# pierlj/ken-burns-effect

Measured on AMD Instinct MI355X. Metric: novel_view_frames_per_sec_1024x1024, higher is better.
Workload: dtype f32; 1 GPU; 1024x1024 KBE path, 1137109 pts (inpaint cloud), frame=shift+scatter+fill+u8+crop/resize; delivery=pinned_host, scatter_route=fused, frames_per_rank=1589, lanes=2, device_only_lanes=4, warmup_frames=3178, passes=1, handoff=sdma, ranks_seen=1

## Files before the change

### include/kbe.h

```cpp
#ifndef KBE_H
#define KBE_H

#include <stddef.h>
#include <stdint.h>

#ifdef __cplusplus
extern "C" {
#endif

#define KBE_ABI_VERSION 11

#if defined(__GNUC__)
#define KBE_API __attribute__((visibility("default")))
#else
#define KBE_API
#endif

enum {
    KBE_OK = 0,
    KBE_E_INVALID = -1,
    KBE_E_LAUNCH = -2,
    KBE_E_DEVICE = -3
};

// ... 87 lines not shown
                                         const double* focals, const float* shifts, void* const* scratch, uint8_t* const* frames_u8,
                                         const int* turns, int placed, int n_next, const double* next_focals, const float* next_shifts,
                                         void* const* next_scratch, const int* next_turns, int stages, const int* fill_rect,
                                         double near_depth, kbe_stream_t stream);

KBE_API int kbe_render_pointcloud_tiled(const float* points, const float* data, int N, int C, int W, int H, double focal,
                                        double baseline, const float* shift3, void* scratch, float* render,
                                        float* existing, kbe_stream_t stream);

#define KBE_MAX_LANES 8
KBE_API size_t kbe_video_scratch_stride(int W, int H, int N);
KBE_API size_t kbe_video_stage_bytes(int W, int H, int lanes, int batch);
#define KBE_VIDEO_FILL_DIST 1
#define KBE_VIDEO_FILL_GROUP(n) (((n) - 1) << 1)
#define KBE_VIDEO_GROUP(n) (((n) - 1) << 5)
#define KBE_VIDEO_FREE_TRANSFERS 8
#define KBE_VIDEO_EVEN_GROUPS 16
#define KBE_VIDEO_NO_AHEAD 512
#define KBE_VIDEO_FAST_RAMP 1024
#define KBE_VIDEO_SDMA 8192
#define KBE_VIDEO_FUSED_LEAN 2048
#define KBE_VIDEO_FUSED_ROOMY 4096
#define KBE_VIDEO_FILL_PAIRS KBE_VIDEO_FILL_GROUP(2)
#define KBE_VIDEO_INJECT_FAULT 32768
#define KBE_VIDEO_INJECT_TIMEOUT 65536
KBE_API int kbe_render_video(const float* points, const float* image, const float* depth, int N, int W, int H,
                             double baseline, int n_frames, const double* focals, const float* shifts, int crop_w,
                             int crop_h, void* scratch, uint8_t* stage, int batch, uint8_t* host_out,
                             int raster_w, int raster_n, const void* packed, double cloud_focal, int flags,
                             kbe_stream_t stream, kbe_stream_t copy_stream, int lanes, const kbe_stream_t* lane_streams,
                             double near_depth);
KBE_API int kbe_video_handoff_status(void);

KBE_API int kbe_generate_mask(const float* points, const float* shift, int B, int N, int W, int H, double focal,
                              double baseline, unsigned long long* keys, int32_t* winner, float* masks, float* zee,
                              int32_t* ids, kbe_stream_t stream);

KBE_API int kbe_frame_u8(const float* render_chw, int W, int H, uint8_t* frame_hwc, kbe_stream_t stream);

KBE_API int kbe_crop_resize_u8(const uint8_t* frame_hwc, int W, int H, int crop_w, int crop_h,
                       uint8_t* out_hwc, kbe_stream_t stream);


KBE_API int kbe_depth_to_points(const float* depth, const float* valid, int B, int W, int H, double focal,
                        float* points, kbe_stream_t stream);

// ... 27 lines not shown
```

### ken-burns-effect_amd/_native.py

```python
import ctypes
import os

import torch

_HERE = os.path.dirname(os.path.abspath(__file__))
LIB_PATH = os.environ.get('KBE_LIB_PATH') or os.path.join(_HERE, 'csrc', 'libkbe_hip.so')

SYMBOLS = (
    'kbe_abi_version', 'kbe_last_error', 'kbe_device_info', 'kbe_selftest_err', 'kbe_selftest_division', 'kbe_zkeys_clear', 'kbe_zsplat', 'kbe_zkeys_decode',
    'kbe_degrid', 'kbe_degrid_serial', 'kbe_accumulate', 'kbe_normalize', 'kbe_render_pointcloud', 'kbe_fill_disocclusion',
    'kbe_frame_scratch_bytes', 'kbe_frame_scratch_init', 'kbe_render_frame', 'kbe_render_frame_stages', 'kbe_render_frame_group', 'kbe_cloud_pack_bytes', 'kbe_cloud_pack', 'kbe_render_frame_fused', 'kbe_render_frame_group_fused', 'kbe_render_frame_group_ahead_ok', 'kbe_render_frame_group_ahead', 'kbe_video_scratch_stride', 'kbe_video_stage_bytes', 'kbe_render_video', 'kbe_render_pointcloud_tiled', 'kbe_generate_mask', 'kbe_frame_u8', 'kbe_crop_resize_u8', 'kbe_depth_to_points', 'kbe_shift_points',
    'kbe_spatial_filter', 'kbe_laplacian_valid', 'kbe_pconv_epilogue', 'kbe_prelu_mask', 'kbe_bias_act', 'kbe_upsample2x_act', 'kbe_frame_scratch_init_sets', 'kbe_video_handoff_status',
)

ABI_VERSION = 11
MAX_LANES = 8
DEFAULT_LANES = 4
FUSED_MAX_DENSITY = 20.0
FUSED_MAX_POINTS = 1 << 28
FUSED_DENSE = 1.5
FUSED_HOST_GROUP = 12
DEFAULT_FILL_GROUP = 4
PROBE_MIN_FRAMES = 128
DEFAULT_HOST_LANES = 2
# ... 516 lines not shown
        if 'stage' not in state or state['stage'].numel() < need:
            state['stage'] = torch.empty(need, dtype=torch.uint8, device=dev)
        if 'copy_stream' not in state:
            state['copy_stream'] = torch.cuda.Stream(device=dev)
            state['lane_streams'] = [None] + lane_streams_of(dev, state['lanes'] - 1)
        lane_streams = (ctypes.c_void_p * MAX_LANES)(*[None if st is None else st.cuda_stream for st in state['lane_streams']])
        focals = (ctypes.c_double * max(n, 1))(*[float(c[0]) for c in cameras])
        shifts = (ctypes.c_float * max(3 * n, 1))(*[float(v) for c in cameras for v in c[1]])
        cw, ch = (0, 0) if crop is None else (int(crop[0]), int(crop[1]))
        copy_stream = ctypes.c_void_p(state['copy_stream'].cuda_stream) if overlap else _stream()
        flags, group, fused = self.video_launch_shape(state, cameras, batch, to_host=not host_out.is_cuda)
        base_flags = flags
        if fused:
            self._pack(state)
        free = os.environ.get('KBE_FREE_TRANSFERS', 'auto')
        if not host_out.is_cuda and (free == '1' or (free == 'auto' and flags & 1)):
            flags |= 8
        if os.environ.get('KBE_EVEN_GROUPS') == '1':
            flags |= 16
        if os.environ.get('KBE_RAMP', 'classic') == 'fast':
            flags |= 1024
        if os.environ.get('KBE_AHEAD') == '0':
            flags |= 512
        flags |= fused_build_bits(video=True)
        if not host_out.is_cuda and batch < 0 and handoff_by_sdma():
            flags |= 8192
            if os.environ.get('KBE_INJECT_HANDOFF_FAULT') == '1':
                flags |= 32768
            if os.environ.get('KBE_INJECT_HANDOFF_TIMEOUT') == '1':
                flags |= 65536
        keep_flags = flags & ~base_flags
        scratch = state['scratch']
        if group > 1:
            fits = group
            if 'scratch_groups' not in state or state['scratch_groups'].numel() < group * lanes * self.scratch_stride(state) or os.environ.get('KBE_SCRATCH_BUDGET_MB'):
                max_sets = self.scratch_set_budget(state)
                while fits > 1 and fits * lanes > max_sets:
                    fits = max(1, fits // 2)
            if fits != group:
                flags, group, fused = self.video_launch_shape(state, cameras, batch, to_host=not host_out.is_cuda, max_group=fits)
                flags |= keep_flags
        state['video_sets'] = group * lanes
        if group > 1:
            scratch, _ = self.group_scratch(state, group * lanes)
        self._check(self.lib.kbe_render_video(_ptr(state['points']), _ptr(state['image']), _ptr(state['depth']), _i(state['N']),
                                              _i(W), _i(H), _d(float(baseline)), _i(n), focals, shifts, _i(cw), _i(ch),
# ... 183 lines not shown
```

### ken-burns-effect_amd/csrc/kbe_fill.h

```cpp
#pragma once
#include <hip/hip_runtime.h>
#include <math.h>

#pragma clang fp contract(off)

namespace kbe {

struct FillDirs { float x[16], y[16]; };

inline FillDirs make_fill_dirs()
{
    const float dx[16] = { -1, 0, 1, 1, -1, 1, 2, 2, -2, -1, 1, 2, 3, 3, 3, 3 };
    const float dy[16] = { 1, 1, 1, 0, 2, 2, 1, -1, 3, 3, 3, 3, 2, 1, -1, -2 };
    FillDirs d;
    for (int i = 0; i < 16; i++) {
        volatile float n = sqrtf((dx[i] * dx[i]) + (dy[i] * dy[i]));
        d.x[i] = dx[i] / n;
        d.y[i] = dy[i] / n;
    }
    return d;
}

template <class DepthAt>
__device__ __forceinline__ int fill_source(const FillDirs& dirs, int x, int y, int W, int H, DepthAt depth_at)
{
// ... 14 lines not shown
        if ((iax < 0) | (iax >= W) | (iay < 0) | (iay >= H)) continue;
        float bx = (float) x, by = (float) y;
        int ibx, iby;
        float db = 0.0f;
        for (;;) {
            bx += ddx; ibx = (int) roundf(bx);
            by += ddy; iby = (int) roundf(by);
            if ((ibx < 0) | (ibx >= W) | (iby < 0) | (iby >= H)) break;
            db = depth_at(ibx, iby);
            if (db > 0.0f) break;
        }
        if ((ibx < 0) | (ibx >= W) | (iby < 0) | (iby >= H)) continue;
        const float ex = (float) (ibx - iax), ey = (float) (iby - iay);
        const float dist = sqrtf(ex * ex + ey * ey);
        if (shortest > dist) {
            fx = iax; fy = iay;
            if (da < db) { fx = ibx; fy = iby; }
            shortest = dist;
        }
    }
    return (fx < 0 || fy < 0) ? -1 : fy * W + fx;
}


}
```

### ken-burns-effect_amd/csrc/kbe_frame.hip

```cpp
#include <stdlib.h>
#include <string.h>

#include <chrono>
#include <mutex>
#include <thread>
#include <vector>
#include <hsa/hsa.h>
#include <hsa/hsa_ext_amd.h>

#include "kbe_cloud.h"
#include "kbe_tiles.h"
#include "kbe_video_plan.h"

using namespace kbe;

namespace {

__global__ void k_scratch_init(uint32_t* zkeys, uint32_t* zkeys_b, size_t hw, int* tile_count, int n_tiles, int* hole_count)
{
    const size_t stride = (size_t) gridDim.x * blockDim.x, gtid = (size_t) blockIdx.x * blockDim.x + threadIdx.x;
    for (size_t i = gtid; i < hw; i += stride) { zkeys[i] = KBE_ZKEY_EMPTY; if (zkeys_b) zkeys_b[i] = KBE_ZKEY_EMPTY; }
    for (size_t i = gtid; i < (size_t) n_tiles; i += stride) { tile_count[i * CNT_STRIDE] = 0; tile_count[i * CNT_STRIDE + 1] = 0; }
    if (gtid < (size_t) HOLE_COUNT_INTS) hole_count[gtid] = 0;
}
// ... 1194 lines not shown
        const hipError_t e = hipMemsetAsync(stage + ctl_offset, 0, sizeof(DeliverCtl), cs);
        if (e != hipSuccess) return fail(KBE_E_LAUNCH, "kbe_render_video: hipMemsetAsync", e);
    }
    if (packed) {
        const Scratch sc0 = carve(scratch, W, H);
        hipLaunchKernelGGL(k_zero_counters, dim3(16, group * lanes), dim3(256), 0, cs, sc0.hole_count, sb, group * lanes, sc0.tile_count,
                           2 * align16(4 * (size_t) sc0.tiles_x * sc0.tiles_y * CNT_STRIDE) / sizeof(int));
        if (int rc0 = launched("kbe_render_video/counters")) return rc0;
    }
    hipEvent_t start = lanes > 1 || (ringed && dc != cs) ? make() : nullptr;
    if (start && ok) {
        (void) hipEventRecord(start, cs);
        for (int l = 1; l < lanes; l++) (void) hipStreamWaitEvent(ls[l], start, 0);
        if (ringed && dc != cs) (void) hipStreamWaitEvent(dc, start, 0);
    }
    const VideoPlan plan = plan_video(VideoPlanIn{ n_frames, lanes, group, batch, dest, fin, (flags & KBE_VIDEO_FAST_RAMP) != 0, (flags & KBE_VIDEO_EVEN_GROUPS) != 0,
                                                   packed != nullptr, !(flags & KBE_VIDEO_NO_AHEAD) },
                                      [&](int n, int n_next) { return fused_can_place_ahead(N, W, H, n, n_next); });

    static const FillDirs fill_dirs = make_fill_dirs();
    const int in_flight = plan.single ? lanes : lanes * group;
    const int fill_flags = in_flight >= KBE_FILL_BY_COUNT_MIN_LANES ? (KBE_STAGE_FILL_BY_COUNT | ((flags & KBE_VIDEO_FILL_DIST) ? KBE_STAGE_FILL_DIST : 0)) : 0;
    const int build = (flags & KBE_VIDEO_FUSED_LEAN) ? 1 : ((flags & KBE_VIDEO_FUSED_ROOMY) ? 2 : 0);
    auto dst = [&](const PlanFrame& f) { return (dest == VideoDest::HBM ? host_out : ringed ? ring0 : finished) + (size_t) f.slot * fb; };
    auto fused_target = [&](const PlanFrame& f, uint8_t* frame) {
        char* const scr = (char*) scratch + (size_t) f.set * sb;
        return FusedTarget{ make_camera(W, H, focals[f.frame], baseline, shifts + 3 * (size_t) f.frame), carve(scr, W, H), scratch_place(scr, W, H), f.turn & 1, frame,
                            nullptr, nullptr, nullptr, nullptr, f.turn };
    };
    auto render = [&](const PlanLaunch& a) {
        const hipStream_t s = ls[a.lane];
        const PlanFrame* const fr = &plan.frames[a.first];
        uint8_t* outs[KBE_FRAME_JOBS];
        uint8_t* raws[KBE_FRAME_JOBS];
        for (int j = 0; j < a.count; j++) {
            outs[j] = dst(fr[j]);
            raws[j] = crop ? stage + (size_t) (KBE_FRAME_JOBS * a.lane + j) * fb : outs[j];
        }
        int rc = KBE_OK;
        if (!packed) {
            FrameJob jobs[KBE_FILL_JOBS];
            for (int j = 0; j < a.count; j++)
                jobs[j] = FrameJob{ focals[fr[j].frame], shifts + 3 * (size_t) fr[j].frame, (char*) scratch + (size_t) fr[j].set * sb, raws[j], nullptr, nullptr, nullptr, nullptr,
                                    fr[j].zbuf == PLAN_ZBUF_A ? KBE_STAGE_ZBUF_A : (fr[j].zbuf == PLAN_ZBUF_B ? KBE_STAGE_ZBUF_B : 0) };
            rc = render_jobs(points, image, depth, N, W, H, baseline, a.count, jobs, KBE_VIDEO_STAGES | fill_flags, crop ? rect : nullptr, raster_w, raster_n, s);
        } else if (plan.single) {
            rc = kbe_render_frame_fused(packed, N, cloud_focal, W, H, focals[fr[0].frame], baseline, shifts + 3 * (size_t) fr[0].frame, (char*) scratch + (size_t) fr[0].set * sb,
                                        raws[0], nullptr, nullptr, nullptr, nullptr, KBE_STAGE_TILES | KBE_STAGE_FILL | fill_flags |
                                        ((flags & KBE_VIDEO_FUSED_LEAN) ? KBE_STAGE_FUSED_LEAN : 0) | ((flags & KBE_VIDEO_FUSED_ROOMY) ? KBE_STAGE_FUSED_ROOMY : 0),
                                        crop ? rect : nullptr, fr[0].turn & 1, (kbe_stream_t) s);
        } else {
            FusedTarget ft[KBE_FRAME_JOBS], nt[KBE_FRAME_JOBS];
            FillTarget targets[KBE_FRAME_JOBS];
            for (int j = 0; j < a.count; j++) {
                ft[j] = fused_target(fr[j], raws[j]);
                targets[j] = FillTarget{ ft[j].sc, ft[j].sc.hole_count + (fr[j].turn & 1), raws[j], nullptr, 0, ft[j].sc.hole_count + ((fr[j].turn & 1) ^ 1) };
            }
            const int n_next = a.next >= 0 ? plan.launches[a.next].count : 0;
            for (int j = 0; j < n_next; j++) nt[j] = fused_target(plan.frames[plan.launches[a.next].first + j], nullptr);
            launch_frames_fused(s, a.count, packed, N, cloud_focal, ft, a.placed, n_next, nt, build, near_depth);
            if ((rc = launched("kbe_render_video/scatter"))) return rc;
            const FillRect fr_rect = { rect[0], rect[1], rect[2], rect[3] };
            for (int j0 = 0; j0 < a.count; j0 += KBE_FILL_JOBS)
                launch_fill(s, a.count - j0 < KBE_FILL_JOBS ? a.count - j0 : KBE_FILL_JOBS, targets + j0, W, H, KBE_STAGE_FILL | fill_flags, fill_dirs, fr_rect,
                            targets[0].sc.tiles_x * targets[0].sc.tiles_y);
            rc = launched("kbe_render_video/fill");
        }
        for (int j0 = 0; j0 < a.count && rc == KBE_OK && crop; j0 += KBE_FILL_JOBS)
            rc = crop_resize_group(a.count - j0 < KBE_FILL_JOBS ? a.count - j0 : KBE_FILL_JOBS, raws + j0, W, H, crop_w, crop_h, outs + j0, s);
        return rc;
    };

    DeliverCtl* const ctl_turns = host_dev && lanes > 1 && !(flags & KBE_VIDEO_FREE_TRANSFERS) ? (DeliverCtl*) (stage + ctl_offset) : nullptr;
    SdmaCall sdma;
    bool sdma_asked = !(flags & KBE_VIDEO_SDMA);
    volatile int64_t* lane_fin[KBE_MAX_LANES] = {};
    const double group_us = (double) -batch * (double) fb / 50.0e3;
    const int turn_polls = (int) fmin(fmax(3.0 * lanes * group_us, (double) DELIVER_MAX_POLLS), 1.0e6);
    hipEvent_t rendered[2][KBE_MAX_LANES] = {}, copied[2] = { nullptr, nullptr };
    for (int h = 0; h < 2 && ringed; h++) {
        copied[h] = make();
        for (int l = 0; l < lanes; l++) if (ls[l] != dc) rendered[h][l] = make();
    }
    if (dest == VideoDest::GROUPS) trace.start((int) plan.units.size(), cs);
    auto wait = [&](int u, const PlanUnit& un) {
        if (dest == VideoDest::GROUPS) {
            trace.begin(u, ls[un.lane]);
            if (lane_fin[un.lane]) hipLaunchKernelGGL(k_signal_wait, dim3(1), dim3(64), 0, ls[un.lane], lane_fin[un.lane], sdma_pool().wait_ticks, sdma_pool().gave_up);
// ... 102 lines not shown
```

### ken-burns-effect_amd/csrc/kbe_hip.hip

```cpp
#include <hip/hip_runtime.h>
#include <math.h>
#include <stdio.h>
#include <string.h>

#include "kbe.h"
#include "kbe_device.h"
#include "kbe_fill.h"
#include "kbe_host.h"

#pragma clang fp contract(off)

using namespace kbe;

thread_local char kbe::g_err[256] = "";

namespace {

__global__ void k_fill_u32(uint32_t* p, size_t n, uint32_t v)
{
    const size_t stride = (size_t) gridDim.x * blockDim.x;
    for (size_t i = (size_t) blockIdx.x * blockDim.x + threadIdx.x; i < n; i += stride) p[i] = v;
}

__global__ void k_zkeys_decode(const uint32_t* keys, size_t n, float* zee)
// ... 226 lines not shown
    s0 = min(max(s, 0), src_n - 1);
    s1 = min(max(s + 1, 0), src_n - 1);
    c0 = cv_round((1.f - f) * 2048.f);
    c1 = cv_round(f * 2048.f);
}

__device__ __forceinline__ uint32_t mul_u24_v(uint32_t a, uint32_t b) { uint32_t r; asm("v_mul_u32_u24 %0, %1, %2" : "=v"(r) : "v"(a), "v"(b)); return r; }
__device__ __forceinline__ uint32_t mad_u24_v(uint32_t a, uint32_t b, uint32_t c) { uint32_t r; asm("v_mad_u32_u24 %0, %1, %2, %3" : "=v"(r) : "v"(a), "v"(b), "v"(c)); return r; }
__device__ __forceinline__ uint32_t mul_u24_s(uint32_t a, uint32_t b) { uint32_t r; asm("v_mul_u32_u24 %0, %1, %2" : "=v"(r) : "s"(a), "v"(b)); return r; }
__device__ __forceinline__ uint32_t mul_hi_u24_s(uint32_t a, uint32_t b) { uint32_t r; asm("v_mul_hi_u32_u24 %0, %1, %2" : "=v"(r) : "s"(a), "v"(b)); return r; }
__device__ __forceinline__ uint32_t mad_u24_s(uint32_t a, uint32_t b, uint32_t c) { uint32_t r; asm("v_mad_u32_u24 %0, %1, %2, %3" : "=v"(r) : "s"(a), "v"(b), "v"(c)); return r; }

#ifndef KBE_CROP_TH
#define KBE_CROP_TH 16
#endif
constexpr int CR_TW = 64, CR_TH = KBE_CROP_TH, CR_THREADS = 256, CR_WAVES = CR_THREADS / 64;
constexpr int CR_ROWS_PER_WAVE = CR_TH / CR_WAVES;
constexpr int CR_PROWS = CR_TH + 2, CR_PCOLS = CR_TW + 2;
constexpr int CR_PBYTES = CR_PCOLS * 3, CR_PSTRIDE = (CR_PBYTES + 3) / 4 + 1;
constexpr int CR_RROWS = CR_PROWS + 1, CR_RDW = ((CR_PCOLS + 1) * 3 + 3 + 3) / 4 + 1;
constexpr int CR_STAGE = (CR_RROWS + CR_WAVES - 1) / CR_WAVES;
static_assert(CR_TH % CR_WAVES == 0 && CR_RDW <= 64 && CR_PBYTES <= CR_THREADS && CR_TW + CR_TH <= CR_THREADS && CR_PROWS + 1 <= CR_THREADS, "crop tile geometry");

__device__ __forceinline__ void crop_resize_body(const uint8_t* __restrict__ img, int W, int H, int cw, int ch_, double scale_x, double scale_y, uint8_t* __restrict__ out)
{
    __shared__ uint32_t s_raw[CR_RROWS][CR_RDW];
    __shared__ uint32_t s_patch[CR_PROWS][CR_PSTRIDE];
    __shared__ __attribute__((aligned(16))) uint32_t s_out[CR_TH][CR_TW * 3 / 4];
    __shared__ int s_cx[4][CR_TW], s_cy[4][CR_TH];
    __shared__ int s_ro[CR_PROWS + 1];
    const int tid = threadIdx.x;
    const int bx = blockIdx.x * CR_TW, by = blockIdx.y * CR_TH;
    const float cx = (float) W / 2.0f - (float) (cw - 1) * 0.5f, cy = (float) H / 2.0f - (float) (ch_ - 1) * 0.5f;
    const int ipx = (int) floorf(cx), ipy = (int) floorf(cy);
    const float fa = cx - (float) ipx, fb = cy - (float) ipy;
    const int a11 = cv_round((1.f - fa) * (1.f - fb) * 65536.f), a12 = cv_round(fa * (1.f - fb) * 65536.f);
    const int a21 = cv_round((1.f - fa) * fb * 65536.f), a22 = cv_round(fa * fb * 65536.f);
    const bool whole = (a12 | a21 | a22) == 0;
    if (tid < CR_TW + CR_TH) {
        const bool col = tid < CR_TW;
        const int k = col ? tid : tid - CR_TW;
        int s0, s1, c0, c1;
        if (col) resize_coeff(min(bx + k, W - 1), scale_x, cw, true, s0, s1, c0, c1);
        else resize_coeff(min(by + k, H - 1), scale_y, ch_, false, s0, s1, c0, c1);
        int* t = col ? &s_cx[0][k] : &s_cy[0][k];
        const int stride = col ? CR_TW : CR_TH;
        t[0] = s0; t[stride] = s1; t[2 * stride] = c0; t[3 * stride] = c1;
    }
    __syncthreads();
    const int px_lo = s_cx[0][0], px_hi = s_cx[1][CR_TW - 1], py_lo = s_cy[0][0], py_hi = s_cy[1][CR_TH - 1];
    const int n_pc3 = (px_hi - px_lo + 1) * 3, n_pr = py_hi - py_lo + 1;
    const int rx0 = min(max(ipx + px_lo, 0), W - 1), rx1 = min(max(ipx + px_hi + 1, 0), W - 1);
    const int ry0 = min(max(ipy + py_lo, 0), H - 1), ry1 = min(max(ipy + py_hi + 1, 0), H - 1);
    const int n_rows = ry1 - ry0 + 1;
    const size_t frame_bytes = (size_t) W * H * 3;
    const int wv = __builtin_amdgcn_readfirstlane(tid >> 6), ln = tid & 63;
    uint32_t stage[CR_STAGE];
#pragma unroll
    for (int k = 0; k < CR_STAGE; k++) {
        const int r = wv + CR_WAVES * k;
        stage[k] = 0;
        if (r < n_rows) {
            const size_t b0 = ((size_t) (ry0 + r) * W + rx0) * 3, b1 = ((size_t) (ry0 + r) * W + rx1) * 3 + 3;
            const size_t a0 = b0 & ~(size_t) 3;
            const int n_dw = (int) ((b1 - a0 + 3) >> 2);
            const uint8_t* row = img + a0;
            if (a0 + 4 * (size_t) n_dw <= frame_bytes) {
                if (ln < n_dw) stage[k] = ((const uint32_t*) row)[ln];
            } else if (ln < n_dw) {
                for (int t = 0; t < 4; t++) if (a0 + 4 * (size_t) ln + t < frame_bytes) stage[k] |= (uint32_t) row[4 * ln + t] << (8 * t);
            }
        }
    }
#pragma unroll
    for (int k = 0; k < CR_STAGE; k++) {
        const int r = wv + CR_WAVES * k;
        if (r < CR_RROWS && ln < CR_RDW) s_raw[r][ln] = stage[k];
    }
    if (tid <= CR_PROWS) {
        const int y = min(max(ipy + py_lo + tid, 0), H - 1);
        s_ro[tid] = min(y - ry0, CR_RROWS - 1) * (int) sizeof(s_raw[0]) + (int) ((((uint32_t) y * (uint32_t) W + (uint32_t) rx0) * 3u) & 3u);
    }
    __syncthreads();
    const uint8_t* raw = (const uint8_t*) s_raw;
    uint8_t* patch = (uint8_t*) s_patch;
    if (!whole) {
        if (tid < n_pc3) {
            const int pc = tid / 3, c = tid - pc * 3;
            const int x0 = (min(max(ipx + px_lo + pc, 0), W - 1) - rx0) * 3 + c, x1 = (min(max(ipx + px_lo + pc + 1, 0), W - 1) - rx0) * 3 + c;
            int o = s_ro[0];
            int t0 = raw[o + x0], t1 = raw[o + x1];
            for (int pr = 0; pr < n_pr; pr++) {
                o = s_ro[pr + 1];
                const int u0 = raw[o + x0], u1 = raw[o + x1];
                const uint32_t t = mad_u24_s((uint32_t) a22, (uint32_t) u1, mad_u24_s((uint32_t) a21, (uint32_t) u0, mad_u24_s((uint32_t) a12, (uint32_t) t1, mad_u24_s((uint32_t) a11, (uint32_t) t0, 1u << 15))));
                patch[pr * (int) sizeof(s_patch[0]) + tid] = (uint8_t) (t >> 16);
                t0 = u0; t1 = u1;
            }
        }
        __syncthreads();
    }
    const int col = tid & (CR_TW - 1);
    const uint8_t* const src = whole ? raw : (const uint8_t*) patch;
    int sx, sx1;
    if (whole) {
        sx = (min(max(ipx + s_cx[0][col], 0), W - 1) - rx0) * 3;
// ... 48 lines not shown
            if (by + r < H) ((uint4*) (out + ((size_t) (by + r) * W + bx) * 3))[k] = ((const uint4*) s_out[r])[k];
        }
    } else if ((W & 3) == 0 && bx + CR_TW <= W) {
        constexpr int DW = CR_TW * 3 / 4;
        for (int i = tid; i < CR_TH * DW; i += CR_THREADS) {
            const int r = i / DW, k = i - r * DW;
            if (by + r < H) ((uint32_t*) (out + ((size_t) (by + r) * W + bx) * 3))[k] = s_out[r][k];
        }
    } else {
#pragma unroll
        for (int m = 0; m < CR_ROWS_PER_WAVE; m++) {
            const int dx = bx + col, dy = by + wv * CR_ROWS_PER_WAVE + m;
            if (dx < W && dy < H) {
                const size_t o = ((size_t) dy * W + dx) * 3;
                out[o] = px[m][0]; out[o + 1] = px[m][1]; out[o + 2] = px[m][2];
            }
        }
    }
}

__global__ void __launch_bounds__(CR_THREADS) k_crop_resize_u8(const uint8_t* __restrict__ img, int W, int H, int cw, int ch_, double scale_x, double scale_y,
                                                               uint8_t* __restrict__ out)
{
    crop_resize_body(img, W, H, cw, ch_, scale_x, scale_y, out);
}

struct CropJobs { const uint8_t* img[4]; uint8_t* out[4]; };
__global__ void __launch_bounds__(CR_THREADS) k_crop_resize_u8_group(CropJobs jobs, int W, int H, int cw, int ch_, double scale_x, double scale_y)
{
    crop_resize_body(jobs.img[blockIdx.z], W, H, cw, ch_, scale_x, scale_y, jobs.out[blockIdx.z]);
}


__device__ __forceinline__ float linspace_centered(int n, int i)
{
    const float start = (float) ((-0.5 * n) + 0.5), end = (float) ((0.5 * n) - 0.5);
    if (n == 1) return start;
    const float step = (end - start) / (float) (n - 1);
    return (i < n / 2) ? start + step * (float) i : end - step * (float) (n - 1 - i);
}

__global__ void __launch_bounds__(kBlock) k_depth_to_points(const float* __restrict__ depth, const float* __restrict__ valid,
                                                            int W, int H, float inv_focal, float* __restrict__ points)
{
    const int b = blockIdx.y;
    const int HW = W * H;
    const int i = blockIdx.x * blockDim.x + threadIdx.x;
    if (i >= HW) return;
    const int y = i / W, x = i - y * W;
    float d = depth[(size_t) b * HW + i];
    if (valid) d = d * valid[(size_t) b * HW + i];
    const float u = linspace_centered(W, x) * inv_focal;
    const float v = linspace_centered(H, y) * inv_focal;
// ... 352 lines not shown
}

int kbe_crop_resize_u8(const uint8_t* frame_hwc, int W, int H, int crop_w, int crop_h, uint8_t* out_hwc,
                       kbe_stream_t stream)
{
    KBE_REQUIRE(frame_hwc && out_hwc && W > 0 && H > 0 && crop_w > 0 && crop_h > 0 && crop_w <= W && crop_h <= H,
                "kbe_crop_resize_u8: bad arguments");
    hipLaunchKernelGGL(k_crop_resize_u8, dim3((W + CR_TW - 1) / CR_TW, (H + CR_TH - 1) / CR_TH), dim3(CR_THREADS), 0,
                       (hipStream_t) stream, frame_hwc, W, H, crop_w, crop_h, (double) crop_w / W, (double) crop_h / H, out_hwc);
    return launched("kbe_crop_resize_u8");
}

}

namespace kbe {
int crop_resize_group(int n, const uint8_t* const* frames, int W, int H, int crop_w, int crop_h, uint8_t* const* outs, hipStream_t stream)
{
    if (n == 1) return kbe_crop_resize_u8(frames[0], W, H, crop_w, crop_h, outs[0], (kbe_stream_t) stream);
    CropJobs jobs;
    for (int k = 0; k < 4; k++) { jobs.img[k] = frames[k < n ? k : 0]; jobs.out[k] = outs[k < n ? k : 0]; }
    hipLaunchKernelGGL(k_crop_resize_u8_group, dim3((W + CR_TW - 1) / CR_TW, (H + CR_TH - 1) / CR_TH, n), dim3(CR_THREADS), 0, stream, jobs, W, H, crop_w, crop_h, (double) crop_w / W, (double) crop_h / H);
    return launched("kbe_crop_resize_u8 (group)");
}
}

extern "C" {

int kbe_depth_to_points(const float* depth, const float* valid, int B, int W, int H, double focal, float* points,
                        kbe_stream_t stream)
{
    KBE_REQUIRE(depth && points && B > 0 && W > 0 && H > 0, "kbe_depth_to_points: bad arguments");
    const float inv = (float) (1.0 / focal);
    hipLaunchKernelGGL(k_depth_to_points, dim3(blocks_for((size_t) W * H), B), dim3(kBlock), 0, (hipStream_t) stream, depth,
                       valid, W, H, inv, points);
    return launched("kbe_depth_to_points");
}

int kbe_shift_points(const float* points, int B, int N, const float* shift3, float* out, kbe_stream_t stream)
{
    KBE_REQUIRE(shift3 && B > 0 && N >= 0, "kbe_shift_points: bad arguments");
    if (N == 0) return KBE_OK;
    KBE_REQUIRE(points && out, "kbe_shift_points: points/out is NULL");
    const Camera cam = make_camera(1, 1, 1.0, 1.0, shift3);
    hipLaunchKernelGGL(k_shift_points, dim3(blocks_for(N), B), dim3(kBlock), 0, (hipStream_t) stream, points, N, cam, out);
    return launched("kbe_shift_points");
}
// ... 68 lines not shown
```

### ken-burns-effect_amd/csrc/kbe_holes.hip

```cpp
#include "kbe_tiles.h"

using namespace kbe;

namespace {


#ifndef KBE_FILL_SERIAL_BATCH
#define KBE_FILL_SERIAL_BATCH 8
#endif
constexpr int COARSE_WORDS = 2048;
#ifndef KBE_FILL_SERIAL_MIN
#define KBE_FILL_SERIAL_MIN 49152
#endif

__device__ __forceinline__ void fill_hole_serial(int px, const float* __restrict__ depth, const uint32_t* __restrict__ mask, int W, int H,
                                                 int wpr, const FillDirs& dirs, int bx0, int by0, int bx1, int by1,
                                                 uint8_t* __restrict__ frame, float* __restrict__ render,
                                                 const uint32_t* near, int c_wpr)
{
    constexpr int SB = KBE_FILL_SERIAL_BATCH;
    static_assert(SB <= 8, "a skipped batch must stay within one 8 x 8 block of where it ends");
    auto far_from_valid = [&](int px_, int py_) { return !((near[(py_ >> 3) * c_wpr + (px_ >> 8)] >> ((px_ >> 3) & 31)) & 1u); };
    const int y = px / W, x = px - y * W;
    float best = 1000000.0f;
// ... 412 lines not shown

#ifndef KBE_FILL_TABLES_BLOCKS
#define KBE_FILL_TABLES_BLOCKS 768
#endif
#ifndef KBE_FILL_BURST
#define KBE_FILL_BURST 4
#endif
#ifndef KBE_FILL_BURST_LANES
#define KBE_FILL_BURST_LANES 16
#endif
#ifndef KBE_FILL_REFILL_MIN
#define KBE_FILL_REFILL_MIN 16
#endif
#ifndef KBE_FILL_FINE_BELOW
#define KBE_FILL_FINE_BELOW 2
#endif
constexpr unsigned long long FILL_NO_ENTRY = ~0ull;
constexpr int FILL_MAX_STEPS = (1 << 14) - 1;
enum { END_IDLE = 0, END_WALK = 1, END_HIT = 2, END_DEAD = 3 };

__device__ __forceinline__ int swap_with_neighbour(int v)
{
    return __builtin_amdgcn_update_dpp(0, v, 0xB1, 0xF, 0xF, false);
}

__device__ __forceinline__ void valid_box(const int4* __restrict__ bbox, int n_tiles, int W, int H, int (*s_bb)[4], int& bx0, int& by0, int& bx1, int& by1)
{
    bx0 = W; by0 = H; bx1 = -1; by1 = -1;
    for (int t = threadIdx.x; t < n_tiles; t += blockDim.x) {
        const int4 bb = bbox[t];
        bx0 = min(bx0, bb.x); by0 = min(by0, bb.y); bx1 = max(bx1, bb.z); by1 = max(by1, bb.w);
    }
#pragma unroll
    for (int off = 32; off > 0; off >>= 1) {
        bx0 = min(bx0, __shfl_xor(bx0, off)); by0 = min(by0, __shfl_xor(by0, off));
        bx1 = max(bx1, __shfl_xor(bx1, off)); by1 = max(by1, __shfl_xor(by1, off));
    }
    if ((threadIdx.x & 63) == 0) { s_bb[threadIdx.x >> 6][0] = bx0; s_bb[threadIdx.x >> 6][1] = by0; s_bb[threadIdx.x >> 6][2] = bx1; s_bb[threadIdx.x >> 6][3] = by1; }
    __syncthreads();
    for (int w = 0; w < (int) (blockDim.x >> 6); w++) { bx0 = min(bx0, s_bb[w][0]); by0 = min(by0, s_bb[w][1]); bx1 = max(bx1, s_bb[w][2]); by1 = max(by1, s_bb[w][3]); }
}

#if defined(KBE_FILL_TABLES_WAVES)
#define KBE_FILL_TABLES_ATTR __attribute__((amdgpu_waves_per_eu(KBE_FILL_TABLES_WAVES, KBE_FILL_TABLES_WAVES)))
#else
#define KBE_FILL_TABLES_ATTR
#endif
__device__ __forceinline__ void fill_tables_body(const int* __restrict__ holes, const int* __restrict__ hole_count, int min_holes,
                                                     const float* __restrict__ depth, int W, int H, FillDirs dirs, FillRect rect,
                                                     uint8_t* __restrict__ frame, float* __restrict__ render, int n_tiles,
                                                     const int4* __restrict__ bbox, int tiles_x, int tiles_y,
                                                     const uint8_t* __restrict__ dist, const float2* __restrict__ strips,
                                                     const uint8_t* __restrict__ dist_blocks)
{
    const int n = min(*hole_count, W * H);
    if (n < min_holes || (int) (blockIdx.x * blockDim.x) >= n) return;
    __shared__ int s_bb[4][4];
    static_assert(KBE_DIST_CAP_BLOCKS <= 15, "block distances are stored in 4 bits");
    __shared__ uint32_t s_pool[COARSE_WORDS];
    int bx0, by0, bx1, by1;
    valid_box(bbox, n_tiles, W, H, s_bb, bx0, by0, bx1, by1);
    constexpr int FB = 256;
    static_assert(FB % 64 == 0 && FB * 16 <= 65536, "queue entries are 16 bits");
// ... 296 lines not shown
                }
                s_near[idx] = near;
            }
            __syncthreads();
        }
        const int gtid = blockIdx.x * blockDim.x + threadIdx.x, gsz = gridDim.x * blockDim.x;
        for (int h = gtid; h < n; h += gsz) {
            const int px = holes[h];
            const int y = px / W, x = px - y * W;
            if (x < rect.x0 || x > rect.x1 || y < rect.y0 || y > rect.y1) continue;
            fill_hole_serial(px, depth, mask, W, H, wpr, dirs, bx0, by0, bx1, by1, frame, render, skip_ok ? s_near : nullptr, c_wpr);
        }
        return;
    }
    const int lane = threadIdx.x & 31;
    const int group = (blockIdx.x * blockDim.x + threadIdx.x) >> 5, n_groups = (gridDim.x * blockDim.x) >> 5;
    const int d = lane >> 1, end = lane & 1;
    const float ddx = end ? dirs.x[d] : -dirs.x[d], ddy = end ? dirs.y[d] : -dirs.y[d];
    const size_t HW = (size_t) W * H;
    for (int h = group; h < n; h += n_groups) {
        const int px = holes[h];
        const int y = px / W, x = px - y * W;
        if (x < rect.x0 || x > rect.x1 || y < rect.y0 || y > rect.y1) continue;
        float fx = (float) x, fy = (float) y;
        int ix = 0, iy = 0;
        bool ok = false;
        bool done = (x < bx0 && ddx <= 0.0f) || (x > bx1 && ddx >= 0.0f) || (y < by0 && ddy <= 0.0f) || (y > by1 && ddy >= 0.0f);
        done = done || (bool) __shfl_xor((int) done, 1);
        auto walk = [&](auto batch_tag) {
            constexpr int kBatch = decltype(batch_tag)::value;
            int bx[kBatch], by[kBatch];
            uint32_t bw[kBatch];
            bool bin[kBatch];
#pragma unroll
            for (int k = 0; k < kBatch; k++) {
                fx += ddx; bx[k] = (int) roundf(fx);
                fy += ddy; by[k] = (int) roundf(fy);
                bin[k] = ((unsigned) bx[k] < (unsigned) W) & ((unsigned) by[k] < (unsigned) H);
                const unsigned mi = bin[k] ? (unsigned) by[k] * (unsigned) wpr + ((unsigned) bx[k] >> 5) : 0u;
                bw[k] = mask[mi];
            }
            bool stop = false;
#pragma unroll
            for (int k = 0; k < kBatch; k++) {
                const bool hit = bin[k] && ((bw[k] >> (bx[k] & 31)) & 1u);
                const bool take = !stop;
                ix = take ? bx[k] : ix; iy = take ? by[k] : iy;
                ok = ok || (take && hit);
                stop = stop || hit || !bin[k];
            }
            done = stop || (ix < bx0 && ddx <= 0.0f) || (ix > bx1 && ddx >= 0.0f) || (iy < by0 && ddy <= 0.0f) || (iy > by1 && ddy >= 0.0f);
        };
        int ox = 0, oy = 0;
        bool ook = false;
        float dist = INFINITY, best = INFINITY;
        for (;;) {
            if (!done) walk(std::integral_constant<int, 8>());
            ox = __shfl_xor(ix, 1); oy = __shfl_xor(iy, 1);
            ook = (bool) __shfl_xor((int) ok, 1);
            const bool odone = (bool) __shfl_xor((int) done, 1);
            const float ex = (float) (ix - ox), ey = (float) (iy - oy);
            const float cur = sqrtf(ex * ex + ey * ey);
            dist = (ok && ook && 1000000.0f > cur) ? cur : INFINITY;
            best = dist;
#pragma unroll
            for (int off = 2; off < 32; off <<= 1) best = fminf(best, __shfl_xor(best, off));
            done = done || (odone && !ook) || cur > best;
            if (__all(done)) break;
        }
        if (best == INFINITY) continue;
        const unsigned long long m = __ballot(dist == best);
        const unsigned mine = (unsigned) (m >> (threadIdx.x & 32));
        const int win = __ffs((int) mine) - 1;
        if (lane == win) {
            int sxp = ix, syp = iy;
            if (depth[(size_t) iy * W + ix] < depth[(size_t) oy * W + ox]) { sxp = ox; syp = oy; }
            const size_t s = (size_t) syp * W + sxp, o = (size_t) px;
            frame[o * 3] = frame[s * 3]; frame[o * 3 + 1] = frame[s * 3 + 1]; frame[o * 3 + 2] = frame[s * 3 + 2];
            if (render) for (int c = 0; c < 4; c++) render[c * HW + o] = render[c * HW + s];
        }
    }
}


}

namespace {

__global__ void __launch_bounds__(256) k_hole_dist(FillJobs jobs, int W, int H, int min_holes, int tiles_x, int tiles_y, FillDirs dirs, int image_rows, int use_strips)
{
    const FillJob& J = jobs.j[blockIdx.z];
    hole_dist_body(J.mask, W, H, J.dist, J.hole_count, min_holes, J.bbox, tiles_x, tiles_y, use_strips ? J.strips : nullptr, dirs, J.coarse, J.dist_blocks, image_rows);
}

__global__ void __launch_bounds__(256) KBE_FILL_TABLES_ATTR k_fill_tables(FillJobs jobs, int min_holes, int W, int H, FillDirs dirs, FillRect rect, int n_tiles,
                                                                         int tiles_x, int tiles_y, int use_strips)
{
    const FillJob& J = jobs.j[blockIdx.y];
    fill_tables_body(J.holes, J.hole_count, min_holes, J.depth, W, H, dirs, rect, J.frame, J.render, n_tiles, J.bbox, tiles_x, tiles_y, J.dist,
// ... 61 lines not shown
```

Measured before the change: 17800 frames/s.

## Fuse disocclusion fill into the crop-resize kernel for video frames

Adds a fused fill+crop/resize kernel. It gathers hole pixels from the validity mask into shared memory per tile, runs the half-wave ray walk to find a source pixel, and patches the staged raw rows before resampling. This replaces the separate fill kernel launch and its full-frame read-modify-write of the u8 frame when cropping is active. The walk logic is factored into a shared helper, and an env flag restores the old path. One risk is that fill sources are read from the unfilled image, so a hole filled from another hole may differ from the sequential path.

```diff
diff --git a/include/kbe.h b/include/kbe.h
--- a/include/kbe.h
+++ b/include/kbe.h
@@ -133,6 +133,7 @@
 #define KBE_VIDEO_FUSED_LEAN 2048
 #define KBE_VIDEO_FUSED_ROOMY 4096
 #define KBE_VIDEO_FILL_PAIRS KBE_VIDEO_FILL_GROUP(2)
+#define KBE_VIDEO_SEPARATE_FILL 16384
 #define KBE_VIDEO_INJECT_FAULT 32768
 #define KBE_VIDEO_INJECT_TIMEOUT 65536
 KBE_API int kbe_render_video(const float* points, const float* image, const float* depth, int N, int W, int H,
diff --git a/ken-burns-effect_amd/_native.py b/ken-burns-effect_amd/_native.py
--- a/ken-burns-effect_amd/_native.py
+++ b/ken-burns-effect_amd/_native.py
@@ -562,6 +562,8 @@
             flags |= 1024
         if os.environ.get('KBE_AHEAD') == '0':
             flags |= 512
+        if os.environ.get('KBE_FILL_CROP') == '0':
+            flags |= 16384
         flags |= fused_build_bits(video=True)
         if not host_out.is_cuda and batch < 0 and handoff_by_sdma():
             flags |= 8192
diff --git a/ken-burns-effect_amd/csrc/kbe_fill.h b/ken-burns-effect_amd/csrc/kbe_fill.h
--- a/ken-burns-effect_amd/csrc/kbe_fill.h
+++ b/ken-burns-effect_amd/csrc/kbe_fill.h
@@ -1,6 +1,8 @@
 #pragma once
 #include <hip/hip_runtime.h>
 #include <math.h>
+#include <stdint.h>
+#include <type_traits>
 
 #pragma clang fp contract(off)
 
@@ -61,5 +63,89 @@
     return (fx < 0 || fy < 0) ? -1 : fy * W + fx;
 }
 
+__device__ __forceinline__ void valid_box(const int4* __restrict__ bbox, int n_tiles, int W, int H, int (*s_bb)[4], int& bx0, int& by0, int& bx1, int& by1)
+{
+    bx0 = W; by0 = H; bx1 = -1; by1 = -1;
+    for (int t = threadIdx.x; t < n_tiles; t += blockDim.x) {
+        const int4 bb = bbox[t];
+        bx0 = min(bx0, bb.x); by0 = min(by0, bb.y); bx1 = max(bx1, bb.z); by1 = max(by1, bb.w);
+    }
+#pragma unroll
+    for (int off = 32; off > 0; off >>= 1) {
+        bx0 = min(bx0, __shfl_xor(bx0, off)); by0 = min(by0, __shfl_xor(by0, off));
+        bx1 = max(bx1, __shfl_xor(bx1, off)); by1 = max(by1, __shfl_xor(by1, off));
+    }
+    if ((threadIdx.x & 63) == 0) { s_bb[threadIdx.x >> 6][0] = bx0; s_bb[threadIdx.x >> 6][1] = by0; s_bb[threadIdx.x >> 6][2] = bx1; s_bb[threadIdx.x >> 6][3] = by1; }
+    __syncthreads();
+    for (int w = 0; w < (int) (blockDim.x >> 6); w++) { bx0 = min(bx0, s_bb[w][0]); by0 = min(by0, s_bb[w][1]); bx1 = max(bx1, s_bb[w][2]); by1 = max(by1, s_bb[w][3]); }
+}
+
+__device__ __forceinline__ bool halfwave_fill_source(int x, int y, float ddx, float ddy, const float* __restrict__ depth, const uint32_t* __restrict__ mask,
+                                                     int W, int H, int wpr, int bx0, int by0, int bx1, int by1, int& sx, int& sy)
+{
+    float fx = (float) x, fy = (float) y;
+    int ix = 0, iy = 0;
+    bool ok = false;
+    bool done = (x < bx0 && ddx <= 0.0f) || (x > bx1 && ddx >= 0.0f) || (y < by0 && ddy <= 0.0f) || (y > by1 && ddy >= 0.0f);
+    done = done || (bool) __shfl_xor((int) done, 1);
+    auto walk = [&](auto batch_tag) {
+        constexpr int kBatch = decltype(batch_tag)::value;
+        int bx[kBatch], by[kBatch];
+        uint32_t bw[kBatch];
+        bool bin[kBatch];
+#pragma unroll
+        for (int k = 0; k < kBatch; k++) {
+            fx += ddx; bx[k] = (int) roundf(fx);
+            fy += ddy; by[k] = (int) roundf(fy);
+            bin[k] = ((unsigned) bx[k] < (unsigned) W) & ((unsigned) by[k] < (unsigned) H);
+            const unsigned mi = bin[k] ? (unsigned) by[k] * (unsigned) wpr + ((unsigned) bx[k] >> 5) : 0u;
+            bw[k] = mask[mi];
+        }
+        bool stop = false;
+#pragma unroll
+        for (int k = 0; k < kBatch; k++) {
+            const bool hit = bin[k] && ((bw[k] >> (bx[k] & 31)) & 1u);
+            const bool take = !stop;
+            ix = take ? bx[k] : ix; iy = take ? by[k] : iy;
+            ok = ok || (take && hit);
+            stop = stop || hit || !bin[k];
+        }
+        done = stop || (ix < bx0 && ddx <= 0.0f) || (ix > bx1 && ddx >= 0.0f) || (iy < by0 && ddy <= 0.0f) || (iy > by1 && ddy >= 0.0f);
+    };
+    int ox = 0, oy = 0;
+    bool ook = false;
+    float dist = INFINITY, best = INFINITY;
+    for (;;) {
+        if (!done) walk(std::integral_constant<int, 8>());
+        ox = __shfl_xor(ix, 1); oy = __shfl_xor(iy, 1);
+        ook = (bool) __shfl_xor((int) ok, 1);
+        const bool odone = (bool) __shfl_xor((int) done, 1);
+        const float ex = (float) (ix - ox), ey = (float) (iy - oy);
+        const float cur = sqrtf(ex * ex + ey * ey);
+        dist = (ok && ook && 1000000.0f > cur) ? cur : INFINITY;
+        best = dist;
+#pragma unroll
+        for (int off = 2; off < 32; off <<= 1) best = fminf(best, __shfl_xor(best, off));
+        done = done || (odone && !ook) || cur > best;
+        if (__all(done)) break;
+    }
+    if (best == INFINITY) return false;
+    const unsigned long long m = __ballot(dist == best);
+    const unsigned mine = (unsigned) (m >> (threadIdx.x & 32));
+    const int win = __ffs((int) mine) - 1;
+    if ((int) (threadIdx.x & 31) != win) return false;
+    sx = ix; sy = iy;
+    if (depth[(size_t) iy * W + ix] < depth[(size_t) oy * W + ox]) { sx = ox; sy = oy; }
+    return true;
+}
+
+struct FillCropJobs {
+    const uint8_t* img[4]; uint8_t* out[4];
+    const uint32_t* mask[4]; const float* depth[4]; const int4* bbox[4];
+    const int* hole_count[4];
+    int* next_hole_count[4];
+};
+int fill_crop_group(int n, const FillCropJobs& jobs, int W, int H, int crop_w, int crop_h, int4 rect, int n_tiles, const FillDirs& dirs, hipStream_t stream);
+
 
 }
diff --git a/ken-burns-effect_amd/csrc/kbe_frame.hip b/ken-burns-effect_amd/csrc/kbe_frame.hip
--- a/ken-burns-effect_amd/csrc/kbe_frame.hip
+++ b/ken-burns-effect_amd/csrc/kbe_frame.hip
@@ -1240,6 +1240,7 @@
     const int in_flight = plan.single ? lanes : lanes * group;
     const int fill_flags = in_flight >= KBE_FILL_BY_COUNT_MIN_LANES ? (KBE_STAGE_FILL_BY_COUNT | ((flags & KBE_VIDEO_FILL_DIST) ? KBE_STAGE_FILL_DIST : 0)) : 0;
     const int build = (flags & KBE_VIDEO_FUSED_LEAN) ? 1 : ((flags & KBE_VIDEO_FUSED_ROOMY) ? 2 : 0);
+    const bool fill_crop = crop && !(flags & (KBE_VIDEO_FILL_DIST | KBE_VIDEO_SEPARATE_FILL));
     auto dst = [&](const PlanFrame& f) { return (dest == VideoDest::HBM ? host_out : ringed ? ring0 : finished) + (size_t) f.slot * fb; };
     auto fused_target = [&](const PlanFrame& f, uint8_t* frame) {
         char* const scr = (char*) scratch + (size_t) f.set * sb;
@@ -1278,10 +1279,25 @@
             for (int j = 0; j < n_next; j++) nt[j] = fused_target(plan.frames[plan.launches[a.next].first + j], nullptr);
             launch_frames_fused(s, a.count, packed, N, cloud_focal, ft, a.placed, n_next, nt, build, near_depth);
             if ((rc = launched("kbe_render_video/scatter"))) return rc;
+            const int n_tiles = targets[0].sc.tiles_x * targets[0].sc.tiles_y;
+            if (fill_crop) {
+                for (int j0 = 0; j0 < a.count && rc == KBE_OK; j0 += KBE_FILL_JOBS) {
+                    const int m = a.count - j0 < KBE_FILL_JOBS ? a.count - j0 : KBE_FILL_JOBS;
+                    FillCropJobs jobs;
+                    for (int k = 0; k < 4; k++) {
+                        const int j = j0 + (k < m ? k : 0);
+                        const FillTarget& t = targets[j];
+                        jobs.img[k] = raws[j]; jobs.out[k] = outs[j];
+                        jobs.mask[k] = t.sc.mask; jobs.depth[k] = t.sc.depth; jobs.bbox[k] = t.sc.bbox;
+                        jobs.hole_count[k] = t.hole_count; jobs.next_hole_count[k] = t.next_hole_count;
+                    }
+                    rc = fill_crop_group(m, jobs, W, H, crop_w, crop_h, make_int4(rect[0], rect[1], rect[2], rect[3]), n_tiles, fill_dirs, s);
+                }
+                return rc;
+            }
             const FillRect fr_rect = { rect[0], rect[1], rect[2], rect[3] };
             for (int j0 = 0; j0 < a.count; j0 += KBE_FILL_JOBS)
-                launch_fill(s, a.count - j0 < KBE_FILL_JOBS ? a.count - j0 : KBE_FILL_JOBS, targets + j0, W, H, KBE_STAGE_FILL | fill_flags, fill_dirs, fr_rect,
-                            targets[0].sc.tiles_x * targets[0].sc.tiles_y);
+                launch_fill(s, a.count - j0 < KBE_FILL_JOBS ? a.count - j0 : KBE_FILL_JOBS, targets + j0, W, H, KBE_STAGE_FILL | fill_flags, fill_dirs, fr_rect, n_tiles);
             rc = launched("kbe_render_video/fill");
         }
         for (int j0 = 0; j0 < a.count && rc == KBE_OK && crop; j0 += KBE_FILL_JOBS)
diff --git a/ken-burns-effect_amd/csrc/kbe_hip.hip b/ken-burns-effect_amd/csrc/kbe_hip.hip
--- a/ken-burns-effect_amd/csrc/kbe_hip.hip
+++ b/ken-burns-effect_amd/csrc/kbe_hip.hip
@@ -272,7 +272,15 @@
 constexpr int CR_STAGE = (CR_RROWS + CR_WAVES - 1) / CR_WAVES;
 static_assert(CR_TH % CR_WAVES == 0 && CR_RDW <= 64 && CR_PBYTES <= CR_THREADS && CR_TW + CR_TH <= CR_THREADS && CR_PROWS + 1 <= CR_THREADS, "crop tile geometry");
 
-__device__ __forceinline__ void crop_resize_body(const uint8_t* __restrict__ img, int W, int H, int cw, int ch_, double scale_x, double scale_y, uint8_t* __restrict__ out)
+struct StagedFill {
+    const uint32_t* mask; const float* depth; const int4* bbox;
+    int n_tiles; int4 rect; float ddx, ddy; bool any;
+};
+constexpr int CR_FILL_COLS = CR_PCOLS + 2;
+
+template <bool kFill>
+__device__ __forceinline__ void crop_resize_body(const uint8_t* __restrict__ img, int W, int H, int cw, int ch_, double scale_x, double scale_y, uint8_t* __restrict__ out,
+                                                 const StagedFill& fill)
 {
     __shared__ uint32_t s_raw[CR_RROWS][CR_RDW];
     __shared__ uint32_t s_patch[CR_PROWS][CR_PSTRIDE];
@@ -297,6 +305,9 @@
         const int stride = col ? CR_TW : CR_TH;
         t[0] = s0; t[stride] = s1; t[2 * stride] = c0; t[3 * stride] = c1;
     }
+    __shared__ uint16_t s_hole[kFill ? CR_RROWS * CR_FILL_COLS : 1];
+    __shared__ int s_n_holes;
+    if (kFill && tid == 0) s_n_holes = 0;
     __syncthreads();
     const int px_lo = s_cx[0][0], px_hi = s_cx[1][CR_TW - 1], py_lo = s_cy[0][0], py_hi = s_cy[1][CR_TH - 1];
     const int n_pc3 = (px_hi - px_lo + 1) * 3, n_pr = py_hi - py_lo + 1;
@@ -327,11 +338,43 @@
         const int r = wv + CR_WAVES * k;
         if (r < CR_RROWS && ln < CR_RDW) s_raw[r][ln] = stage[k];
     }
+    if constexpr (kFill) {
+        const int wpr = (W + 31) >> 5;
+        const int xa = max(rx0, fill.rect.x), xb = min(rx1, fill.rect.z);
+        const int r = tid >> 2, wi = (xa >> 5) + (tid & 3), y = ry0 + r;
+        if (fill.any && tid < CR_RROWS * 4 && r < n_rows && y >= fill.rect.y && y <= fill.rect.w && xa <= xb && wi <= (xb >> 5)) {
+            const int lo = max(xa - 32 * wi, 0), hi = min(xb - 32 * wi, 31);
+            uint32_t h = ~fill.mask[(size_t) y * wpr + wi] & (0xFFFFFFFFu << lo) & (0xFFFFFFFFu >> (31 - hi));
+            if (h) {
+                int at = atomicAdd(&s_n_holes, __popc(h));
+                for (; h; h &= h - 1) s_hole[at++] = (uint16_t) ((r << 8) | (32 * wi + __ffs((int) h) - 1 - rx0));
+            }
+        }
+    }
     if (tid <= CR_PROWS) {
         const int y = min(max(ipy + py_lo + tid, 0), H - 1);
         s_ro[tid] = min(y - ry0, CR_RROWS - 1) * (int) sizeof(s_raw[0]) + (int) ((((uint32_t) y * (uint32_t) W + (uint32_t) rx0) * 3u) & 3u);
     }
     __syncthreads();
+    if constexpr (kFill) {
+        const int n_holes = s_n_holes;
+        if (n_holes > 0) {
+            __shared__ int s_bb[CR_WAVES][4];
+            int bx0, by0, bx1, by1;
+            valid_box(fill.bbox, fill.n_tiles, W, H, s_bb, bx0, by0, bx1, by1);
+            const int wpr = (W + 31) >> 5;
+            for (int h = tid >> 5; h < n_holes; h += CR_THREADS / 32) {
+                const int e = s_hole[h], r = e >> 8, x = rx0 + (e & 255), y = ry0 + r;
+                int sx, sy;
+                if (halfwave_fill_source(x, y, fill.ddx, fill.ddy, fill.depth, fill.mask, W, H, wpr, bx0, by0, bx1, by1, sx, sy)) {
+                    const uint8_t* s = img + ((size_t) sy * W + sx) * 3;
+                    uint8_t* o = (uint8_t*) s_raw[r] + (x - rx0) * 3 + (int) ((((uint32_t) y * (uint32_t) W + (uint32_t) rx0) * 3u) & 3u);
+                    o[0] = s[0]; o[1] = s[1]; o[2] = s[2];
+                }
+            }
+            __syncthreads();
+        }
+    }
     const uint8_t* raw = (const uint8_t*) s_raw;
     uint8_t* patch = (uint8_t*) s_patch;
     if (!whole) {
@@ -426,13 +469,24 @@
 __global__ void __launch_bounds__(CR_THREADS) k_crop_resize_u8(const uint8_t* __restrict__ img, int W, int H, int cw, int ch_, double scale_x, double scale_y,
                                                                uint8_t* __restrict__ out)
 {
-    crop_resize_body(img, W, H, cw, ch_, scale_x, scale_y, out);
+    crop_resize_body<false>(img, W, H, cw, ch_, scale_x, scale_y, out, StagedFill{});
 }
 
 struct CropJobs { const uint8_t* img[4]; uint8_t* out[4]; };
 __global__ void __launch_bounds__(CR_THREADS) k_crop_resize_u8_group(CropJobs jobs, int W, int H, int cw, int ch_, double scale_x, double scale_y)
 {
-    crop_resize_body(jobs.img[blockIdx.z], W, H, cw, ch_, scale_x, scale_y, jobs.out[blockIdx.z]);
+    crop_resize_body<false>(jobs.img[blockIdx.z], W, H, cw, ch_, scale_x, scale_y, jobs.out[blockIdx.z], StagedFill{});
+}
+
+__global__ void __launch_bounds__(CR_THREADS) k_fill_crop_u8_group(FillCropJobs jobs, int W, int H, int cw, int ch_, double scale_x, double scale_y,
+                                                                   int4 rect, int n_tiles, FillDirs dirs)
+{
+    const int z = blockIdx.z;
+    if (jobs.next_hole_count[z] && blockIdx.x == 0 && blockIdx.y == 0 && threadIdx.x == 0) *jobs.next_hole_count[z] = 0;
+    const int d = (threadIdx.x & 31) >> 1, end = threadIdx.x & 1;
+    const StagedFill fill{ jobs.mask[z], jobs.depth[z], jobs.bbox[z], n_tiles, rect, end ? dirs.x[d] : -dirs.x[d], end ? dirs.y[d] : -dirs.y[d],
+                           *jobs.hole_count[z] > 0 };
+    crop_resize_body<true>(jobs.img[z], W, H, cw, ch_, scale_x, scale_y, jobs.out[z], fill);
 }
 
 
@@ -831,6 +885,14 @@
     hipLaunchKernelGGL(k_crop_resize_u8_group, dim3((W + CR_TW - 1) / CR_TW, (H + CR_TH - 1) / CR_TH, n), dim3(CR_THREADS), 0, stream, jobs, W, H, crop_w, crop_h, (double) crop_w / W, (double) crop_h / H);
     return launched("kbe_crop_resize_u8 (group)");
 }
+
+int fill_crop_group(int n, const FillCropJobs& jobs, int W, int H, int crop_w, int crop_h, int4 rect, int n_tiles, const FillDirs& dirs, hipStream_t stream)
+{
+    KBE_REQUIRE(n >= 1 && n <= 4 && W > 0 && H > 0 && crop_w > 0 && crop_h > 0 && crop_w <= W && crop_h <= H, "fill_crop_group: bad arguments");
+    hipLaunchKernelGGL(k_fill_crop_u8_group, dim3((W + CR_TW - 1) / CR_TW, (H + CR_TH - 1) / CR_TH, n), dim3(CR_THREADS), 0, stream, jobs, W, H, crop_w, crop_h,
+                       (double) crop_w / W, (double) crop_h / H, rect, n_tiles, dirs);
+    return launched("kbe_fill_crop_u8 (group)");
+}
 }
 
 extern "C" {
diff --git a/ken-burns-effect_amd/csrc/kbe_holes.hip b/ken-burns-effect_amd/csrc/kbe_holes.hip
--- a/ken-burns-effect_amd/csrc/kbe_holes.hip
+++ b/ken-burns-effect_amd/csrc/kbe_holes.hip
@@ -458,23 +458,6 @@
 __device__ __forceinline__ int swap_with_neighbour(int v)
 {
     return __builtin_amdgcn_update_dpp(0, v, 0xB1, 0xF, 0xF, false);
-}
-
-__device__ __forceinline__ void valid_box(const int4* __restrict__ bbox, int n_tiles, int W, int H, int (*s_bb)[4], int& bx0, int& by0, int& bx1, int& by1)
-{
-    bx0 = W; by0 = H; bx1 = -1; by1 = -1;
-    for (int t = threadIdx.x; t < n_tiles; t += blockDim.x) {
-        const int4 bb = bbox[t];
-        bx0 = min(bx0, bb.x); by0 = min(by0, bb.y); bx1 = max(bx1, bb.z); by1 = max(by1, bb.w);
-    }
-#pragma unroll
-    for (int off = 32; off > 0; off >>= 1) {
-        bx0 = min(bx0, __shfl_xor(bx0, off)); by0 = min(by0, __shfl_xor(by0, off));
-        bx1 = max(bx1, __shfl_xor(bx1, off)); by1 = max(by1, __shfl_xor(by1, off));
-    }
-    if ((threadIdx.x & 63) == 0) { s_bb[threadIdx.x >> 6][0] = bx0; s_bb[threadIdx.x >> 6][1] = by0; s_bb[threadIdx.x >> 6][2] = bx1; s_bb[threadIdx.x >> 6][3] = by1; }
-    __syncthreads();
-    for (int w = 0; w < (int) (blockDim.x >> 6); w++) { bx0 = min(bx0, s_bb[w][0]); by0 = min(by0, s_bb[w][1]); bx1 = max(bx1, s_bb[w][2]); by1 = max(by1, s_bb[w][3]); }
 }
 
 #if defined(KBE_FILL_TABLES_WAVES)
@@ -817,59 +800,8 @@
         const int px = holes[h];
         const int y = px / W, x = px - y * W;
         if (x < rect.x0 || x > rect.x1 || y < rect.y0 || y > rect.y1) continue;
-        float fx = (float) x, fy = (float) y;
-        int ix = 0, iy = 0;
-        bool ok = false;
-        bool done = (x < bx0 && ddx <= 0.0f) || (x > bx1 && ddx >= 0.0f) || (y < by0 && ddy <= 0.0f) || (y > by1 && ddy >= 0.0f);
-        done = done || (bool) __shfl_xor((int) done, 1);
-        auto walk = [&](auto batch_tag) {
-            constexpr int kBatch = decltype(batch_tag)::value;
-            int bx[kBatch], by[kBatch];
-            uint32_t bw[kBatch];
-            bool bin[kBatch];
-#pragma unroll
-            for (int k = 0; k < kBatch; k++) {
-                fx += ddx; bx[k] = (int) roundf(fx);
-                fy += ddy; by[k] = (int) roundf(fy);
-                bin[k] = ((unsigned) bx[k] < (unsigned) W) & ((unsigned) by[k] < (unsigned) H);
-                const unsigned mi = bin[k] ? (unsigned) by[k] * (unsigned) wpr + ((unsigned) bx[k] >> 5) : 0u;
-                bw[k] = mask[mi];
-            }
-            bool stop = false;
-#pragma unroll
-            for (int k = 0; k < kBatch; k++) {
-                const bool hit = bin[k] && ((bw[k] >> (bx[k] & 31)) & 1u);
-                const bool take = !stop;
-                ix = take ? bx[k] : ix; iy = take ? by[k] : iy;
-                ok = ok || (take && hit);
-                stop = stop || hit || !bin[k];
-            }
-            done = stop || (ix < bx0 && ddx <= 0.0f) || (ix > bx1 && ddx >= 0.0f) || (iy < by0 && ddy <= 0.0f) || (iy > by1 && ddy >= 0.0f);
-        };
-        int ox = 0, oy = 0;
-        bool ook = false;
-        float dist = INFINITY, best = INFINITY;
-        for (;;) {
-            if (!done) walk(std::integral_constant<int, 8>());
-            ox = __shfl_xor(ix, 1); oy = __shfl_xor(iy, 1);
-            ook = (bool) __shfl_xor((int) ok, 1);
-            const bool odone = (bool) __shfl_xor((int) done, 1);
-            const float ex = (float) (ix - ox), ey = (float) (iy - oy);
-            const float cur = sqrtf(ex * ex + ey * ey);
-            dist = (ok && ook && 1000000.0f > cur) ? cur : INFINITY;
-            best = dist;
-#pragma unroll
-            for (int off = 2; off < 32; off <<= 1) best = fminf(best, __shfl_xor(best, off));
-            done = done || (odone && !ook) || cur > best;
-            if (__all(done)) break;
-        }
-        if (best == INFINITY) continue;
-        const unsigned long long m = __ballot(dist == best);
-        const unsigned mine = (unsigned) (m >> (threadIdx.x & 32));
-        const int win = __ffs((int) mine) - 1;
-        if (lane == win) {
-            int sxp = ix, syp = iy;
-            if (depth[(size_t) iy * W + ix] < depth[(size_t) oy * W + ox]) { sxp = ox; syp = oy; }
+        int sxp, syp;
+        if (halfwave_fill_source(x, y, ddx, ddy, depth, mask, W, H, wpr, bx0, by0, bx1, by1, sxp, syp)) {
             const size_t s = (size_t) syp * W + sxp, o = (size_t) px;
             frame[o * 3] = frame[s * 3]; frame[o * 3 + 1] = frame[s * 3 + 1]; frame[o * 3 + 2] = frame[s * 3 + 2];
             if (render) for (int c = 0; c < 4; c++) render[c * HW + o] = render[c * HW + s];
```

Measured after the change: 17810 frames/s (median of 4 runs). Within noise of the previous version (+0.1%).
